# Tariq-Abuhashim/semantic-slam

Measured on AMD Instinct MI355X. Metric: Mvoxels/sec integrated, 512³ grid @ 640×480 depth; achieved HBM GB/s %peak, higher is better.
Workload: dtype f32

## Files before the change

### semantic_slam_amd/csrc/tsdf_capi.hip

```cpp
#include "../../include/tsdf_hip.h"

#include <hip/hip_runtime.h>

#include <algorithm>
#include <cmath>
#include <cstdarg>
#include <cstdio>
#include <cstdlib>
#include <cstring>
#include <new>
#include <string>
#include <unordered_map>
#include <vector>

#include "pose_math.h"
#include "host_derive.h"
#include "host_copy.h"
#include "frame_store.h"
#include "tsdf_kernels.hip.h"
#include "tsdf_multiframe.hip.h"
#include "tsdf_labels.hip.h"
#include "tsdf_colour.hip.h"
#include "tsdf_extract.hip.h"
#ifdef TSDF_EXPERIMENTS
#include "tsdf_experiments.hip.h"
#endif

namespace {

thread_local std::string g_last_error;

int fail(int code, const char *fmt, ...)
{
    char buf[512];
    va_list ap;
    va_start(ap, fmt);
    vsnprintf(buf, sizeof buf, fmt, ap);
    va_end(ap);
    g_last_error = buf;
    return code;
}

#define HIP_TRY(expr)                                                                          \
    do {                                                                                       \
        hipError_t _e = (expr);                                                                \
        if (_e != hipSuccess)                                                                  \
            return fail(TSDF_ERR_HIP, "%s failed: %s (%s:%d)", #expr, hipGetErrorString(_e),   \
                        __FILE__, __LINE__);                                                   \
    } while (0)

constexpr int kStageSlots = 3;

#ifdef TSDF_EXPERIMENTS
constexpr bool kExperiments = true;
#else
constexpr bool kExperiments = false;
#endif

#ifndef TSDF_BRICK_NT
#define TSDF_BRICK_NT 0
#endif
constexpr bool kBrickNT = TSDF_BRICK_NT != 0;
constexpr size_t kClaimBlockBytes = (tsdfk::kCounterBytes + sizeof(tsdfk::ClassPoseTable) + 255) / 256 * 256;
#ifndef TSDF_WEDGE_MODE
#define TSDF_WEDGE_MODE 0
#endif
constexpr int kWedgeMode = TSDF_WEDGE_MODE;

}

struct tsdf_volume {
    tsdf_config cfg;
    float base2world_inv[16];
    float last_cam2base[16];
    int64_t n_vox;
    float *d_tsdf;
    float *d_weight;
    hipStream_t own_stream;
    hipStream_t stream;
    tsdf_store::FrameStore *store;
    hipStream_t copy_stream;
    hipEvent_t flush_done[2];
    int flush_parity;
    int table_slot;
    int defer_n;
    hipEvent_t pend_copied;
    int pend_count;
    int pend_slot[tsdfk::kMaxFramesPerLaunch], pend_mask_slot[tsdfk::kMaxFramesPerLaunch];
    const float *pend_depth[tsdfk::kMaxFramesPerLaunch];
    struct tsdf_batch *owner;
    struct tsdf_group *group_owner;
    bool in_flush;
    float pend_c2b[16 * tsdfk::kMaxFramesPerLaunch];
    const uint8_t *pend_mask[tsdfk::kMaxFramesPerLaunch];
    int variant;
    tsdfk::FramePose *h_frames[kStageSlots];
    tsdfk::FramePose *d_frames[kStageSlots];
    hipEvent_t frames_done[kStageSlots];
    bool frames_used[kStageSlots];
    int frames_next;
    uint16_t *d_label;
    float *d_fp, *d_bp;
    float prob_thd;
    uint32_t *d_colour;
    uint8_t *d_rgb[kStageSlots];
    uint8_t *h_rgb[kStageSlots];
    hipEvent_t rgb_done[kStageSlots];
    bool rgb_used[kStageSlots];
    int rgb_next;
    uint32_t *d_flags;
    size_t n_flags;
    int nseg;
    int chunks_per_slice;
    bool flat;
    int brick_q, brick_r, brick_s;
    int tile;
    bool fine_tables = false;
    bool flags_known_zero;
    unsigned int *d_super;
    size_t super_words;
    uint4 *d_work;
    size_t work_entries;
    int64_t work_nsuper, work_bucket_supers;
    int work_wedge_mode = -1;
    unsigned int *d_shortcut_stats;
    unsigned long long *d_claims, *h_claims;
    hipEvent_t claims_done;
    hipStream_t pre_stream = nullptr, rb_stream = nullptr;
    int rb_parity = -1;
    hipEvent_t pre_done[2] = {nullptr, nullptr}, list_free[2] = {nullptr, nullptr}, seq_ready = nullptr;
    int list_parity = 0;
    bool list_used[2] = {false, false};
    bool pipeline_ok = false;
    bool claims_pending, claims_known;
    double claims_total;
    double claim_fraction;
    int launches_unclassified;
    void *d_scratch;
    size_t scratch_bytes;
    uint8_t *d_wg_class;
    size_t wg_class_bytes;
    void *d_list;
    size_t list_bytes;
};

constexpr int kBatchSideStreams = 4;

struct tsdf_batch {
    int device;
    std::vector<tsdf_volume *> vols;
    hipStream_t stream;
    tsdfk::IntegrateParams *h_params[kStageSlots];
    tsdfk::IntegrateParams *d_params[kStageSlots];
    tsdfk::FramePose *h_poses[kStageSlots];
    tsdfk::FramePose *d_poses[kStageSlots];
    hipEvent_t slot_done[kStageSlots];
    bool slot_used[kStageSlots];
    int slot_next;
    int2 *d_slice_map;
    int total_slices, max_blocks;
    int2 *d_group_map;
    int total_groups;
    std::vector<int> group_s;
    float2 *d_tiles;
    size_t tiles_per_object;
    uint8_t *d_wg_class;
    uint8_t *d_brick_class;
    size_t brick_class_bytes;
    float *d_depth_pool;
    uint8_t *d_mask_pool;
    std::vector<float> pend_c2b;
    std::vector<const uint8_t *> pend_mask;
    int pend_count;
    bool in_flush;
    hipStream_t side[kBatchSideStreams];
    hipEvent_t side_done[kBatchSideStreams];
    hipEvent_t collected;
};

namespace {

int flush_pending(tsdf_volume *v);
int fail(int code, const char *fmt, ...);
int batch_flush(tsdf_batch *b);
int group_flush(tsdf_group *g);
int batch_collect(tsdf_batch *b, const float *depth_dev, const uint8_t *const *masks_dev, const float cam2world[16]);

int bind_device(tsdf_volume *v, bool flush = true)
{
    HIP_TRY(hipSetDevice(v->cfg.device));
    if (v->owner && !v->in_flush) {
        int rc = batch_flush(v->owner);
        if (rc) return rc;
    }
    if (v->group_owner && !v->in_flush) {
        int rc = group_flush(v->group_owner);
        if (rc) return rc;
    }
    if (flush && v->pend_count > 0 && !v->in_flush) return flush_pending(v);
    return TSDF_OK;
}

int store_slot(tsdf_volume *v, tsdf_store::SlotClass *c, hipStream_t first_user, int *index, void **dev)
{
    hipError_t e = tsdf_store::slot_acquire(v->store, c, v, first_user, false, index, dev);
    if (e == hipSuccess && *index < 0) {
        if (v->pend_count > 0 && !v->in_flush) {
            int rc = flush_pending(v);
            if (rc) return rc;
        }
        e = tsdf_store::slot_acquire(v->store, c, v, first_user, true, index, dev);
    }
    if (e != hipSuccess) return fail(TSDF_ERR_HIP, "frame store: %s", hipGetErrorString(e));
    return TSDF_OK;
}

int store_release(tsdf_volume *v, tsdf_store::SlotClass *c, const int *idx, int n)
{
    hipEvent_t *evt = &v->flush_done[v->flush_parity];
    HIP_TRY(hipEventRecord(*evt, v->stream));
    tsdf_store::slots_release_after(v->store, c, idx, n, evt, v);
    return TSDF_OK;
}

void store_next_pass(tsdf_volume *v) { v->flush_parity ^= 1; }

int tables_begin(tsdf_volume *v, float2 **tiles, hipStream_t first_user = nullptr)
{
    void *dev = nullptr;
    hipError_t e = tsdf_store::slot_acquire(v->store, &v->store->tables, v, first_user ? first_user : v->stream, true, &v->table_slot, &dev);
    if (e != hipSuccess) return fail(TSDF_ERR_HIP, "frame store (tile tables): %s", hipGetErrorString(e));
    *tiles = static_cast<float2 *>(dev);
    return TSDF_OK;
}

int tables_end(tsdf_volume *v)
{
    if (v->table_slot < 0) return TSDF_OK;
    const int slot = v->table_slot;
    v->table_slot = -1;
    return store_release(v, &v->store->tables, &slot, 1);
}

using tsdf_host::brick_shape_ok;

void choose_brick_for(const tsdf_config &c, int &bq, int &br, int &bs)
{
#ifdef TSDF_EXPERIMENTS
// ... 77 lines not shown

size_t tile_table_elems_host(int tiles_w, int tiles_h)
{
    return (size_t)tile_levels_host(tiles_w) * tile_levels_host(tiles_h) * tiles_w * tiles_h;
}

bool tiles_fit(const tsdfk::IntegrateParams &p) { return (int64_t)p.tiles_w * p.tiles_h <= 16384; }

constexpr int64_t kFineTileMinVoxels = 10000000;
thread_local bool g_create_for_batch = false;
int tile_edge_for(const tsdf_config &c)
{
    const int64_t n = (int64_t)c.dim_x * c.dim_y * (int64_t)(c.z_end - c.z_begin);
    const int64_t fine_tiles = (int64_t)((c.im_width + 7) / 8) * ((c.im_height + 7) / 8);
    return (!g_create_for_batch && n >= kFineTileMinVoxels && fine_tiles <= tsdfk::kTileLdsEntries) ? 8 : 16;
}

constexpr int64_t kFineLevelMinVoxels = 64000000;
bool fine_tables_for(const tsdf_config &c, int tile)
{
    const int64_t n = (int64_t)c.dim_x * c.dim_y * (int64_t)(c.z_end - c.z_begin);
    bool on = tile == 8 && n >= kFineLevelMinVoxels;
#ifdef TSDF_EXPERIMENTS
    if (const char *e = std::getenv("TSDF_FINE_TILES")) on = tile == 8 && std::atoi(e) != 0;
#endif
    return on;
}

constexpr int64_t kClassifyMinVoxels = 48000000;
bool classify_one_frame(const tsdf_volume *v, int64_t launch_voxels)
{
    if (v->variant == 7) return false;
    return v->variant == 8 || (kExperiments && v->variant >= 11 && v->variant <= 13) || launch_voxels >= kClassifyMinVoxels;
}

int build_tile_tables(hipStream_t stream, const tsdf_config &c, const tsdfk::IntegrateParams &p, const float *const *depth,
                      const uint8_t *const *masks, int n, float2 *tables, unsigned long long *zero_me = nullptr, float2 *fine = nullptr,
                      bool beside_a_launch = false)
{
    const size_t per = tile_table_elems_host(p.tiles_w, p.tiles_h);
    if (fine != nullptr && (p.tile_inv != 0.125f || n > tsdfk::kMaxFramesPerLaunch))
        return fail(TSDF_ERR_INVALID, "build_tile_tables: fine tables go with 8-pixel tiles, one launch at a time");
    for (int k = 0; k < n; k += tsdfk::kMaxFramesPerLaunch) {
        const int m = std::min(tsdfk::kMaxFramesPerLaunch, n - k);
        tsdfk::TileSummaryParams tp;
        for (int f = 0; f < tsdfk::kMaxFramesPerLaunch; ++f) {
            tp.depth[f] = depth[k + (f < m ? f : 0)];
            tp.mask[f] = masks ? masks[k + (f < m ? f : 0)] : nullptr;
        }
        tp.tiles = tables + (size_t)k * per;
        tp.H = c.im_height; tp.W = c.im_width; tp.tiles_w = p.tiles_w; tp.tiles_h = p.tiles_h;
        tp.max_depth = c.max_depth;
        tp.fine = fine; tp.fw = p.fine_w; tp.fh = p.fine_h;
        if (p.tile_inv == 0.0625f) {
            const int strips = ((p.tiles_w + 3) / 4) * p.tiles_h;
            hipLaunchKernelGGL(tsdfk::depth_tile_summary<16>, dim3((unsigned)((strips + 3) / 4), m), dim3(64, 4), 0, stream, tp);
        } else {
            const int strips = ((p.tiles_w + 7) / 8) * p.tiles_h;
            hipLaunchKernelGGL(tsdfk::depth_tile_summary<8>, dim3((unsigned)((strips + 3) / 4), m), dim3(64, 4), 0, stream, tp);
        }
        if (p.tiles_w * p.tiles_h <= tsdfk::kTileLdsEntries) {
            const unsigned threads = (p.tiles_w * p.tiles_h > 2048 && !beside_a_launch) ? 1024 : 256;
            const unsigned fine_blocks = fine ? ((unsigned)(p.fine_w * p.fine_h) + threads - 1) / threads : 0u;
            hipLaunchKernelGGL(tsdfk::tile_sparse_table, dim3((unsigned)tile_levels_host(p.tiles_w) + fine_blocks, m), dim3(threads), 0, stream, tp.tiles,
                               p.tiles_w, p.tiles_h, k == 0 ? zero_me : (unsigned long long *)nullptr, fine, p.fine_w, p.fine_h);
        } else {
            if (zero_me && k == 0) HIP_TRY(hipMemsetAsync(zero_me, 0, tsdfk::kCounterBytes, stream));
            hipLaunchKernelGGL(tsdfk::tile_sparse_table_scan, dim3((unsigned)tile_levels_host(p.tiles_w), m), dim3(256), 0, stream, tp.tiles,
                               p.tiles_w, p.tiles_h);
            if (fine)
                hipLaunchKernelGGL(tsdfk::fine_tile_levels, dim3((unsigned)((p.fine_w * p.fine_h + 255) / 256), m), dim3(256), 0, stream, fine, p.fine_w, p.fine_h);
        }
    }
    HIP_TRY(hipGetLastError());
    return TSDF_OK;
}

int launch_masked_bricks(tsdf_volume *v, tsdfk::IntegrateParams &p)
{
    const int blocks = (p.brick_groups * p.bricks_per_group + 3) / 4, nz = (p.nz + p.brick_s - 1) / p.brick_s;
    float2 *tiles = nullptr;
    int rc0 = tables_begin(v, &tiles);
    if (rc0) return rc0;
    const size_t n_bricks = (size_t)blocks * nz * 4;
    if (v->wg_class_bytes < n_bricks) {
        if (v->d_wg_class) HIP_TRY(hipFree(v->d_wg_class));
        v->d_wg_class = nullptr;
        v->wg_class_bytes = 0;
        HIP_TRY(hipMalloc((void **)&v->d_wg_class, n_bricks));
        v->wg_class_bytes = n_bricks;
    }
    const float *d = p.depth;
    const uint8_t *m = p.mask;
    int rc = build_tile_tables(v->stream, v->cfg, p, &d, &m, 1, tiles);
    if (rc) return rc;
    tsdfk::FramePose pose;
    pose_from_params(pose, p);
    pose.tiles = tiles;
    hipLaunchKernelGGL(tsdfk::classify_bricks, dim3((unsigned)((n_bricks + 255) / 256)), dim3(256), 0, v->stream, p, pose,
                       v->d_wg_class, blocks, nz);
    p.wg_class = v->d_wg_class;
    hipLaunchKernelGGL((tsdfk::integrate_single_bricks<kBrickNT>), dim3(blocks, 1, nz), dim3(64, 4, 1), 0, v->stream, p, pose);
    HIP_TRY(hipGetLastError());
    return tables_end(v);
}


bool shipped_variant(int variant) { return variant == 0 || variant == 1 || variant == 3 || variant == 7 || variant == 8; }

int drop_summary(tsdf_volume *v)
{
    if (v->flags_known_zero || v->n_flags == 0) return TSDF_OK;
    HIP_TRY(hipMemsetAsync(v->d_flags, 0, v->n_flags * sizeof(uint32_t), v->stream));
    v->flags_known_zero = true;
    return TSDF_OK;
}

int rebuild_summary(tsdf_volume *v)
{
    if (v->n_flags == 0 || v->n_vox == 0) return TSDF_OK;
    const int nz = v->cfg.z_end - v->cfg.z_begin;
    const int qps = (int)((int64_t)v->cfg.dim_x * v->cfg.dim_y / 4);
    dim3 block(64, 4, 1), grid((v->chunks_per_slice + 3) / 4, 1, nz);
    hipLaunchKernelGGL(tsdfk::recompute_flags, grid, block, 0, v->stream, v->d_tsdf, v->d_weight, v->d_flags, qps,
                       v->chunks_per_slice);
    HIP_TRY(hipGetLastError());
    v->flags_known_zero = false;
    return TSDF_OK;
}

int launch_multi(tsdf_volume *v, const float *const *depth_dev, const uint8_t *const *masks_dev, const float *c2b, int n,
                 const uint16_t *const *label_ims = nullptr, const float *const *score_ims = nullptr, hipEvent_t inputs_ready = nullptr);

double claims_read_back(const tsdf_volume *v)
{
    double claimed = 0.0;
    for (int b = 0; b < tsdfk::kListBuckets; ++b) {
        const unsigned long long w = v->h_claims[(size_t)b * (tsdfk::kBucketStride / sizeof(unsigned long long)) + 1];
        claimed += (double)(w >> 32) + (double)(w & 0xffffffffull);
    }
    return v->claims_total > 0 ? claimed / v->claims_total : 0.0;
}

#ifdef TSDF_EXPERIMENTS
bool experiment_variant(int variant);
void experiment_adjust(const tsdf_volume *v, bool labels, bool *classify, int *z_fastest);
int launch_integrate_experiment(tsdf_volume *v, const float *depth_dev, const uint8_t *mask_dev, const float *c2b);
int launch_multi_experiment(tsdf_volume *v, tsdfk::MultiParamsInline &mi, const float *const *depth_dev, const uint8_t *const *masks_dev,
                            const float *c2b, int n, bool labels, bool any_mask, bool classify, bool *handled, double *claims_total);
int launch_single_experiment(tsdf_volume *v, tsdfk::IntegrateParams &common, tsdfk::FramePose &pose, const float *depth_dev,
                             const float *c2b, bool *handled);
#endif

int launch_integrate(tsdf_volume *v, const float *depth_dev, const uint8_t *mask_dev,
                     const float *c2b)
{
    const tsdf_config &c = v->cfg;
    const int nz = c.z_end - c.z_begin;
    if (nz == 0) return TSDF_OK;
    std::memcpy(v->last_cam2base, c2b, sizeof v->last_cam2base);
#ifdef TSDF_EXPERIMENTS
    if (c.dim_x % 4 == 0 && (v->variant == 2 || (v->variant >= 16 && !mask_dev))) return launch_integrate_experiment(v, depth_dev, mask_dev, c2b);
#endif
    if (c.dim_x % 4 != 0 || v->variant == 1) {
        int rc = drop_summary(v);
        if (rc) return rc;
        const tsdfk::IntegrateParams p = make_params(v, depth_dev, mask_dev, c2b, 1);
        dim3 block(64, 4, 1), grid((c.dim_x + 63) / 64, (c.dim_y + 3) / 4, nz);
        if (mask_dev) hipLaunchKernelGGL((tsdfk::integrate_scalar<true>), grid, block, 0, v->stream, p);
        else hipLaunchKernelGGL((tsdfk::integrate_scalar<false>), grid, block, 0, v->stream, p);
        HIP_TRY(hipGetLastError());
        return TSDF_OK;
    }
    if (v->flat) {
        return launch_multi(v, &depth_dev, mask_dev ? &mask_dev : nullptr, c2b, 1);
    }
    tsdfk::IntegrateParams p = make_params(v, depth_dev, mask_dev, c2b, 4);
    v->flags_known_zero = false;
    const dim3 block(64, 4, 1), grid((p.xgroups + 63) / 64, (p.dim_y + 7) / 8, p.nz);
    if (mask_dev) {
        if (classify_one_frame(v, v->n_vox) && tiles_fit(p) && p.brick_q > 0 && (!kExperiments || v->variant != 11)) {
            int rc = launch_masked_bricks(v, p);
            if (rc) return rc;
        } else {
#ifdef TSDF_EXPERIMENTS
            if (v->variant == 11 && classify_one_frame(v, v->n_vox) && tiles_fit(p)) return launch_integrate_experiment(v, depth_dev, mask_dev, c2b);
#endif
            hipLaunchKernelGGL((tsdfk::integrate_tile<2, true>), grid, block, 0, v->stream, p);
        }
    } else {
        hipLaunchKernelGGL((tsdfk::integrate_tile<2, false>), grid, block, 0, v->stream, p);
    }
    HIP_TRY(hipGetLastError());
    return TSDF_OK;
}

void compose_cam2base(const tsdf_volume *v, const float *cam2world, float *c2b)
{
    tsdf_host::multiply_matrix(v->base2world_inv, cam2world, c2b);
}

int launch_multi(tsdf_volume *v, const float *const *depth_dev, const uint8_t *const *masks_dev,
                 const float *c2b, int n, const uint16_t *const *label_ims, const float *const *score_ims, hipEvent_t inputs_ready)
{
    const tsdf_config &c = v->cfg;
    const int nz = c.z_end - c.z_begin;
    if (nz == 0 || n == 0) return TSDF_OK;
    auto fill_pose = [&](tsdfk::FramePose &fp, int f) {
        pose_from_params(fp, make_params(v, depth_dev[f], masks_dev ? masks_dev[f] : nullptr, c2b + 16 * f, 4));
        fp.label_im = label_ims ? label_ims[f] : nullptr;
        fp.score_im = label_ims ? score_ims[f] : nullptr;
    };
    const dim3 block(64, 4, 1);
    if (n == 1 && !label_ims) {
        tsdfk::IntegrateParams common = make_params(v, depth_dev[0], nullptr, c2b, 4);
        tsdfk::FramePose pose;
        fill_pose(pose, 0);
        std::memcpy(v->last_cam2base, c2b, sizeof v->last_cam2base);
        v->flags_known_zero = false;
#ifdef TSDF_EXPERIMENTS
        {
            bool handled = false;
            int rc = launch_single_experiment(v, common, pose, depth_dev[0], c2b, &handled);
            if (rc || handled) return rc;
        }
#endif
        if (v->flat && pose.mask != nullptr && classify_one_frame(v, v->n_vox) && tiles_fit(common) && common.brick_q > 0) {
            tsdfk::IntegrateParams cp = make_params(v, depth_dev[0], pose.mask, c2b, 4);
            return launch_masked_bricks(v, cp);
        }
        if (v->flat) {
            dim3 grid((v->chunks_per_slice + 3) / 4, 1, nz);
            hipLaunchKernelGGL((tsdfk::integrate_multi_single<true, true>), grid, block, 0, v->stream, common, pose);
        } else {
            dim3 grid((common.xgroups + 63) / 64, (c.dim_y + 3) / 4, nz);
            hipLaunchKernelGGL((tsdfk::integrate_multi_single<true, false>), grid, block, 0, v->stream, common, pose);
        }
        HIP_TRY(hipGetLastError());
        return TSDF_OK;
    }
    std::memcpy(v->last_cam2base, c2b + 16 * (n - 1), sizeof v->last_cam2base);
    v->flags_known_zero = false;
    tsdfk::MultiParamsInline mi;
    mi.common = make_params(v, depth_dev[0], nullptr, c2b, 4);
    mi.n_frames = n;
    for (int f = 0; f < n; ++f) fill_pose(mi.frames[f], f);
    for (int f = n; f < tsdfk::kMaxFramesPerLaunch; ++f) mi.frames[f] = mi.frames[0];
    mi.labels.label = v->d_label; mi.labels.fp = v->d_fp; mi.labels.bp = v->d_bp; mi.labels.prob_thd = v->prob_thd;
    bool any_mask = false;
    for (int f = 0; f < n && masks_dev; ++f) any_mask = any_mask || masks_dev[f] != nullptr;

    if (v->claims_pending) {
        const hipError_t qe = hipEventQuery(v->claims_done);
        if (qe == hipSuccess) {
            v->claim_fraction = claims_read_back(v);
            v->claims_pending = false;
            v->claims_known = true;
        } else if (qe == hipErrorNotReady) {
            (void)hipGetLastError();
        } else {
            v->claims_pending = false;
            v->claims_known = false;
            (void)hipGetLastError();
            return fail(TSDF_ERR_HIP, "claims read-back: hipEventQuery failed: %s", hipGetErrorString(qe));
        }
    }
    bool classify = tiles_fit(mi.common) && v->variant != 7 && mi.common.brick_q > 0;
    mi.z_fastest = 2;
#ifdef TSDF_EXPERIMENTS
    experiment_adjust(v, label_ims != nullptr, &classify, &mi.z_fastest);
#endif
    const bool forced = v->variant == 8 || (kExperiments && v->variant >= 11 && v->variant <= 13);
    if (classify && !forced) classify = !v->claims_known || v->claim_fraction >= 0.10 || v->launches_unclassified >= 7;
    v->launches_unclassified = classify ? 0 : v->launches_unclassified + 1;
    const bool count_claims = classify && !v->claims_pending;
    if (classify && !v->d_claims) {
        unsigned long long *dc = nullptr;
        unsigned char *hc = nullptr;
        hipEvent_t ev[6] = {nullptr, nullptr, nullptr, nullptr, nullptr, nullptr};
        hipError_t e = hipMalloc((void **)&dc, 2 * kClaimBlockBytes);
        if (e == hipSuccess) e = hipHostMalloc((void **)&hc, tsdfk::kCounterBytes, hipHostMallocDefault);
        for (int i = 0; i < 6 && e == hipSuccess; ++i) e = hipEventCreateWithFlags(&ev[i], hipEventDisableTiming);
        if (e != hipSuccess) {
            for (int i = 0; i < 6; ++i) if (ev[i]) (void)hipEventDestroy(ev[i]);
            if (hc) (void)hipHostFree(hc);
            if (dc) (void)hipFree(dc);
            return fail(TSDF_ERR_HIP, "claim counters: %s", hipGetErrorString(e));
        }
        v->d_claims = reinterpret_cast<decltype(v->d_claims)>(dc);
        v->h_claims = reinterpret_cast<decltype(v->h_claims)>(hc);
        v->claims_done = ev[0];
        v->pre_done[0] = ev[1]; v->pre_done[1] = ev[2]; v->list_free[0] = ev[3]; v->list_free[1] = ev[4]; v->seq_ready = ev[5];
    }
    const int P = v->pipeline_ok ? v->list_parity : 0;
    unsigned long long *const claims_p = classify ? v->d_claims + (size_t)P * (kClaimBlockBytes / sizeof(unsigned long long)) : nullptr;
    bool pipelined = classify && inputs_ready != nullptr && v->pipeline_ok;
#ifdef TSDF_EXPERIMENTS
    if (!shipped_variant(v->variant) || std::getenv("TSDF_NO_PIPELINE")) pipelined = false;
#endif
    if (pipelined && !v->pre_stream) {
        hipStream_t a = nullptr, b = nullptr;
        int prio = 0;
#ifdef TSDF_EXPERIMENTS
        if (std::getenv("TSDF_PRE_PRIORITY")) { int lo = 0, hi = 0; (void)hipDeviceGetStreamPriorityRange(&lo, &hi); prio = hi; }
#endif
        hipError_t e = hipStreamCreateWithPriority(&a, hipStreamNonBlocking, prio);
        if (e == hipSuccess) e = hipStreamCreateWithFlags(&b, hipStreamNonBlocking);
        if (e != hipSuccess) {
            if (a) (void)hipStreamDestroy(a);
            return fail(TSDF_ERR_HIP, "side streams: %s", hipGetErrorString(e));
        }
        v->pre_stream = a;
        v->rb_stream = b;
    }
    const hipStream_t ps = pipelined ? v->pre_stream : v->stream;
    if (pipelined) {
        HIP_TRY(hipStreamWaitEvent(ps, inputs_ready, 0));
        if (v->list_used[P]) HIP_TRY(hipStreamWaitEvent(ps, v->list_free[P], 0));
        if (v->rb_parity == P) HIP_TRY(hipStreamWaitEvent(ps, v->claims_done, 0));
    } else if (classify && v->rb_parity == P) {
        HIP_TRY(hipStreamWaitEvent(v->stream, v->claims_done, 0));
    }
    if (count_claims) mi.common.claim_counter = claims_p + 1;
    if (classify) {
        const size_t per_frame = tile_table_elems_host(mi.common.tiles_w, mi.common.tiles_h);
        float2 *tiles = nullptr;
        int rc = tables_begin(v, &tiles, ps);
        if (rc) return rc;
        float2 *fine = v->fine_tables ? tiles + (size_t)tsdfk::kMaxFramesPerLaunch * per_frame : nullptr;
        rc = build_tile_tables(ps, c, mi.common, depth_dev, masks_dev, n, tiles, claims_p, fine, pipelined);
        if (rc) return rc;
        mi.common.fine = fine;
        for (int f = 0; f < n; ++f) mi.frames[f].tiles = tiles + (size_t)f * per_frame;
        for (int f = n; f < tsdfk::kMaxFramesPerLaunch; ++f) mi.frames[f] = mi.frames[0];
    }
    const int nz_groups = (nz + mi.common.brick_s - 1) / mi.common.brick_s;
    double claims_total = 0.0;
    bool launched = false, listed = false;
#ifdef TSDF_EXPERIMENTS
    {
        int rc = launch_multi_experiment(v, mi, depth_dev, masks_dev, c2b, n, label_ims != nullptr, any_mask, classify, &launched, &claims_total);
        if (rc) return rc;
    }
// ... 2066 lines not shown
```

### semantic_slam_amd/csrc/tsdf_kernels.hip.h

```cpp
#pragma once
#include <hip/hip_runtime.h>
#include <stdint.h>

namespace tsdfk {

struct IntegrateParams {
    const float *depth;
    const uint8_t *mask;
    float *tsdf;
    float *weight;
    float fx, fy, cx, cy;
    float rx0, rx1, rx2;
    float ry0, ry1, ry2;
    float rz0, rz1, rz2;
    float tx, ty, tz;
    float ox, oy, oz;
    float vs, trunc, max_depth;
    int dim_x, dim_y;
    int nz, z_begin;
    int H, W;
    int xgroups;
    uint32_t *flags;
    int nseg;
    int quads_per_row, quads_per_slice, chunks_per_slice;
    int brick_q, brick_r, brick_s, bricks_per_group, brick_groups;
    int brick_q_magic, brick_per_magic;
    int fast_ok;
    int trunc_fast;
    float cz_margin;
    int tiles_w, tiles_h;
    float tile_inv;
    const float2 *fine = nullptr;
    int fine_w = 0, fine_h = 0;
    float px_margin_u, px_margin_v;
    unsigned int *shortcut_stats;
    float cz_short, cz_pad;
    unsigned long long *claim_counter;
    const uint8_t *wg_class;
};

struct RowTerms {
    float x1, x2, y1, y2, z1, z2;
};

__device__ __forceinline__ RowTerms row_terms(const IntegrateParams &p, int gy, int gz)
{
    float by = p.oy + (float)gy * p.vs;
    float bz = p.oz + (float)gz * p.vs;
    float dy = by - p.ty;
    float dz = bz - p.tz;
    RowTerms r;
    r.x1 = p.rx1 * dy; r.x2 = p.rx2 * dz;
    r.y1 = p.ry1 * dy; r.y2 = p.ry2 * dz;
    r.z1 = p.rz1 * dy; r.z2 = p.rz2 * dz;
    return r;
}

template <bool MASKED>
__device__ __forceinline__ bool voxel_dist(const IntegrateParams &p, const RowTerms &r, int gx,
                                           float &dist)
{
    float bx = p.ox + (float)gx * p.vs;
    float dx = bx - p.tx;
    float pcx = p.rx0 * dx + r.x1 + r.x2;
    float pcy = p.ry0 * dx + r.y1 + r.y2;
    float pcz = p.rz0 * dx + r.z1 + r.z2;
    if (pcz <= 0.0f) return false;

    float pu = roundf(p.fx * (pcx / pcz) + p.cx);
    float pv = roundf(p.fy * (pcy / pcz) + p.cy);
    if (!(pu >= 0.0f && pu < (float)p.W && pv >= 0.0f && pv < (float)p.H)) return false;
    int pix = (int)pv * p.W + (int)pu;

    float d = p.depth[pix];
    if (MASKED) d = d * (p.mask[pix] >= 128 ? 1.0f : 0.0f);
    if (d <= 0.0f || d > p.max_depth) return false;

    float diff = d - pcz;
    if (diff <= -p.trunc) return false;
    dist = fminf(1.0f, diff / p.trunc);
    return true;
}

template <bool MASKED>
__global__ __launch_bounds__(256) void integrate_scalar(IntegrateParams p)
{
    const int gx = blockIdx.x * 64 + threadIdx.x;
    const int gy = blockIdx.y * 4 + threadIdx.y;
    const int lz = blockIdx.z;
    if (gx >= p.dim_x || gy >= p.dim_y) return;
    const int gz = p.z_begin + lz;
    const RowTerms r = row_terms(p, gy, gz);
    float dist;
    const bool upd = voxel_dist<MASKED>(p, r, gx, dist);
    if (__ballot(upd) == 0ull) return;
    if (!upd) return;
    const size_t at = ((size_t)lz * p.dim_y + gy) * (size_t)p.dim_x + (size_t)gx;
    const float w_old = p.weight[at];
    const float w_new = w_old + 1.0f;
    p.weight[at] = w_new;
    p.tsdf[at] = (p.tsdf[at] * w_old + dist) / w_new;
}

typedef float v2f __attribute__((ext_vector_type(2)));

__device__ __forceinline__ float refined_rcp(float d)
{
    const float r0 = __builtin_amdgcn_rcpf(d);
    const float e0 = __builtin_fmaf(-d, r0, 1.0f);
    return __builtin_fmaf(e0, r0, r0);
}

__device__ __forceinline__ float fast_div_r(float n, float d, float r1)
{
    const float q0 = n * r1;
    const float e1 = __builtin_fmaf(-d, q0, n);
    const float q1 = __builtin_fmaf(e1, r1, q0);
    const float e2 = __builtin_fmaf(-d, q1, n);
    return __builtin_fmaf(e2, r1, q1);
}

__device__ __forceinline__ v2f fast_div2(v2f n, float d)
{
    const float r1 = refined_rcp(d);
    const v2f R = {r1, r1}, D = {d, d};
    const v2f q0 = n * R;
    const v2f e1 = __builtin_elementwise_fma(-D, q0, n);
    const v2f q1 = __builtin_elementwise_fma(e1, R, q0);
    const v2f e2 = __builtin_elementwise_fma(-D, q1, n);
    return __builtin_elementwise_fma(e2, R, q1);
}

__device__ __forceinline__ int round_half_up_i32(float u)
{
    int r;
    asm("v_cvt_rpi_i32_f32 %0, %1" : "=v"(r) : "v"(u));
    return r;
}

#define TSDF_FAST_D_MIN 8.6736174e-19f

typedef float v4f __attribute__((ext_vector_type(4)));
typedef unsigned int v4u __attribute__((ext_vector_type(4)));

template <bool NT>
__device__ __forceinline__ float4 vol_load(const float *p)
{
    if constexpr (NT) {
        v4f v = __builtin_nontemporal_load(reinterpret_cast<const v4f *>(p));
        return make_float4(v.x, v.y, v.z, v.w);
    } else {
        return *reinterpret_cast<const float4 *>(p);
    }
}
template <bool NT>
__device__ __forceinline__ void vol_store(float *p, float4 v)
{
    if constexpr (NT) {
        v4f q = {v.x, v.y, v.z, v.w};
        __builtin_nontemporal_store(q, reinterpret_cast<v4f *>(p));
    } else {
        *reinterpret_cast<float4 *>(p) = v;
    }
}

__device__ __forceinline__ float gather_f32(const float *__restrict__ base, uint32_t px)
{
    return *reinterpret_cast<const float *>(reinterpret_cast<const char *>(base) + (px << 2));
}

__device__ __forceinline__ int pixel_index24(int iv, int W, int iu)
{
    return (int)(__umul24((unsigned)iv, (unsigned)W) + (unsigned)iu);
}

template <int R, int MASKED>
__device__ __forceinline__ void integrate_tile_body(const IntegrateParams &p, const int bx, const int by, const int lz)
{
    const int gz = p.z_begin + lz;
    const int xg = bx * 64 + threadIdx.x;
    const int gy0 = (by * 4 + threadIdx.y) * R;
    if (xg >= p.xgroups || gy0 >= p.dim_y) return;
    const size_t row0 = ((size_t)lz * p.dim_y + gy0) * (size_t)p.dim_x + (size_t)xg * 4;
    const size_t flag0 = ((size_t)lz * p.dim_y + gy0) * (size_t)p.nseg + bx;

    uint32_t fl[R];
    float4 t4[R], w4[R];
#pragma unroll
    for (int r = 0; r < R; ++r) {
        fl[r] = gy0 + r < p.dim_y ? p.flags[flag0 + (size_t)r * p.nseg] : 0u;
        t4[r] = make_float4(1.f, 1.f, 1.f, 1.f);
        w4[r] = make_float4(0.f, 0.f, 0.f, 0.f);
    }

    float ax[4], ay[4], az[4];
#pragma unroll
    for (int j = 0; j < 4; ++j) {
        float bx = p.ox + (float)(xg * 4 + j) * p.vs;
        float dx = bx - p.tx;
        ax[j] = p.rx0 * dx; ay[j] = p.ry0 * dx; az[j] = p.rz0 * dx;
    }
    const float bz = p.oz + (float)gz * p.vs;
    const float dz = bz - p.tz;
    const float x2 = p.rx2 * dz, y2 = p.ry2 * dz, z2 = p.rz2 * dz;

    float pcz[R][4], dval[R][4];
    bool geo[R][4];
    int pixel[R][4];
#pragma unroll
    for (int r = 0; r < R; ++r) {
        const float dy = (p.oy + (float)(gy0 + r) * p.vs) - p.ty;
        const float z1 = p.rz1 * dy;
#pragma unroll
        for (int j = 0; j < 4; ++j) pcz[r][j] = az[j] + z1 + z2;
    }
    const float cmin = fminf(fminf(pcz[0][0], pcz[0][3]), fminf(pcz[R - 1][0], pcz[R - 1][3]));
    const float cmax = fmaxf(fmaxf(pcz[0][0], pcz[0][3]), fmaxf(pcz[R - 1][0], pcz[R - 1][3]));
    const bool unsafe = !(cmin > p.cz_margin) & !(cmax < -p.cz_margin);
    const bool fast = p.fast_ok != 0 && __ballot(unsafe) == 0ull;
    if (fast) {
        const v2f F = {p.fx, p.fy}, C = {p.cx, p.cy};
        const bool front = cmin > p.cz_margin;
#pragma unroll
        for (int r = 0; r < R; ++r) {
            const bool row_ok = gy0 + r < p.dim_y;
            const float dy = (p.oy + (float)(gy0 + r) * p.vs) - p.ty;
            const v2f XY1 = {p.rx1 * dy, p.ry1 * dy};
            const v2f XY2 = {x2, y2};
#pragma unroll
            for (int j = 0; j < 4; ++j) {
                const v2f A = {ax[j], ay[j]};
                const v2f n = A + XY1 + XY2;
                const float cz = pcz[r][j];
                const v2f uv = F * fast_div2(n, cz) + C;
                const int iu = round_half_up_i32(uv.x), iv = round_half_up_i32(uv.y);
                const bool ok = row_ok & front & (uv.x > -0.5f) & (uv.y > -0.5f) &
                                ((unsigned)iu < (unsigned)p.W) & ((unsigned)iv < (unsigned)p.H);
                geo[r][j] = ok;
                pixel[r][j] = ok ? pixel_index24(iv, p.W, iu) : 0;
            }
        }
    } else {
#pragma unroll
        for (int r = 0; r < R; ++r) {
            const int gy = gy0 + r;
            const bool row_ok = gy < p.dim_y;
            const float by = p.oy + (float)gy * p.vs;
            const float dy = by - p.ty;
            const float x1 = p.rx1 * dy, y1 = p.ry1 * dy;
#pragma unroll
            for (int j = 0; j < 4; ++j) {
                const float cx = ax[j] + x1 + x2;
                const float cy = ay[j] + y1 + y2;
                const float cz = pcz[r][j];
                const float pu = roundf(p.fx * (cx / cz) + p.cx);
                const float pv = roundf(p.fy * (cy / cz) + p.cy);
                const bool ok = row_ok && !(cz <= 0.0f) && pu >= 0.0f && pu < (float)p.W && pv >= 0.0f &&
                                pv < (float)p.H;
                geo[r][j] = ok;
                pixel[r][j] = ok ? (int)pv * p.W + (int)pu : 0;
            }
        }
    }
#pragma unroll
    for (int r = 0; r < R; ++r) {
#pragma unroll
        for (int j = 0; j < 4; ++j) {
            const uint32_t px = (uint32_t)pixel[r][j];
            float d = gather_f32(p.depth, px);
            if (MASKED == 1) d = d * (p.mask[px] >= 128 ? 1.0f : 0.0f);
            dval[r][j] = d;
        }
    }

    float diff[R][4];
    bool upd[R][4], rowany[R], bandr[R];
    bool any = false, band = false;
#pragma unroll
    for (int r = 0; r < R; ++r) {
        rowany[r] = false;
        bandr[r] = false;
#pragma unroll
        for (int j = 0; j < 4; ++j) {
            const float d = dval[r][j];
            const float df = d - pcz[r][j];
            diff[r][j] = df;
            const bool u = geo[r][j] & !((d <= 0.0f) | (d > p.max_depth)) & !(df <= -p.trunc);
            upd[r][j] = u;
            rowany[r] |= u;
            bandr[r] |= u & !(df >= p.trunc);
        }
        band |= bandr[r];
        any |= rowany[r];
    }
    if (__ballot(any) == 0ull) return;
    if (!any) return;

#pragma unroll
    for (int r = 0; r < R; ++r) {
        if (rowany[r]) {
            w4[r] = vol_load<true>(p.weight + row0 + (size_t)r * p.dim_x);
            if (!(fl[r] & 1u)) t4[r] = vol_load<true>(p.tsdf + row0 + (size_t)r * p.dim_x);
        }
    }
    float dist[R][4];
    if (__ballot(band) != 0ull) {
#pragma unroll
        for (int r = 0; r < R; ++r)
#pragma unroll
            for (int j = 0; j < 4; ++j) dist[r][j] = fminf(1.0f, diff[r][j] / p.trunc);
    } else {
#pragma unroll
        for (int r = 0; r < R; ++r)
#pragma unroll
            for (int j = 0; j < 4; ++j) dist[r][j] = 1.0f;
    }

#pragma unroll
    for (int r = 0; r < R; ++r) {
        if (fl[r] == 3u && __ballot(bandr[r]) == 0ull) {
            if (rowany[r]) {
                const float4 w = w4[r];
                vol_store<true>(p.weight + row0 + (size_t)r * p.dim_x,
                                make_float4(upd[r][0] ? w.x + 1.0f : w.x, upd[r][1] ? w.y + 1.0f : w.y,
                                            upd[r][2] ? w.z + 1.0f : w.z, upd[r][3] ? w.w + 1.0f : w.w));
            }
            continue;
        }
        float tv[4] = {t4[r].x, t4[r].y, t4[r].z, t4[r].w};
        float wv[4] = {w4[r].x, w4[r].y, w4[r].z, w4[r].w};
        float num[4], wn[4];
        bool need = false;
#pragma unroll
        for (int j = 0; j < 4; ++j) {
            wn[j] = wv[j] + 1.0f;
            num[j] = tv[j] * wv[j] + dist[r][j];
            need |= upd[r][j] && !(num[j] == wn[j] && wn[j] < 3.0e38f && wn[j] > 0.0f);
        }
        float nt[4];
        if (__ballot(rowany[r] && need) != 0ull) {
#pragma unroll
            for (int j = 0; j < 4; ++j) nt[j] = num[j] / wn[j];
        } else {
#pragma unroll
            for (int j = 0; j < 4; ++j) nt[j] = 1.0f;
        }
        bool changed = false, notone = false;
#pragma unroll
        for (int j = 0; j < 4; ++j) {
            const float newt = upd[r][j] ? nt[j] : tv[j];
            changed |= __float_as_uint(newt) != __float_as_uint(tv[j]);
            notone |= upd[r][j] && __float_as_uint(newt) != 0x3f800000u;
            tv[j] = newt;
            wv[j] = upd[r][j] ? wn[j] : wv[j];
        }
        if ((fl[r] & 1u) && __ballot(notone) != 0ull) {
            if (notone) p.flags[flag0 + (size_t)r * p.nseg] = fl[r] & 2u;
        }
        const bool store_t = __ballot(rowany[r] && changed) != 0ull;
        if (rowany[r]) {
            if (store_t) vol_store<true>(p.tsdf + row0 + (size_t)r * p.dim_x, make_float4(tv[0], tv[1], tv[2], tv[3]));
            vol_store<true>(p.weight + row0 + (size_t)r * p.dim_x, make_float4(wv[0], wv[1], wv[2], wv[3]));
        }
    }
}

template <int R, bool MASKED>
__global__ __launch_bounds__(256) void integrate_tile(IntegrateParams p)
{
    integrate_tile_body<R, MASKED ? 1 : 0>(p, blockIdx.x, blockIdx.y, blockIdx.z);
}

__device__ __forceinline__ uint32_t hash32(uint64_t x)
{
    x ^= x >> 33; x *= 0xff51afd7ed558ccdull; x ^= x >> 33; x *= 0xc4ceb9fe1a85ec53ull; x ^= x >> 33;
    return (uint32_t)x;
}

__global__ __launch_bounds__(256) void selftest_fastdiv(uint64_t seed, uint64_t n_samples, float fx, float cx,
                                                        unsigned long long *mismatch, float *first_bad)
{
    const uint64_t stride = (uint64_t)gridDim.x * blockDim.x;
    for (uint64_t i = (uint64_t)blockIdx.x * blockDim.x + threadIdx.x; i < n_samples; i += stride) {
        const uint32_t h0 = hash32(seed + 3 * i), h1 = hash32(seed + 3 * i + 1), h2 = hash32(seed + 3 * i + 2);
        const uint32_t mode = h2 & 7u;
        uint32_t dm = h0 & 0x7fffffu;
        if (mode == 1) dm = 0x7fffffu; else if (mode == 2) dm = 0u; else if (mode == 3) dm &= 0x7u;
        const uint32_t de = 127u - 60u + (h0 >> 23) % 121u;
        const float d = __uint_as_float((de << 23) | dm);
        uint32_t ne = (mode >= 6) ? ((h1 >> 23) % 190u) : (de - 12u + (h1 >> 23) % 24u);
        if (ne > 127u + 60u) ne = 127u + 60u;
        uint32_t nm = h1 & 0x7fffffu;
        if (mode == 4) nm = 0x7fffffu; else if (mode == 5) nm = dm;
        float n0 = __uint_as_float(((h2 >> 3) & 1u) << 31 | (ne << 23) | nm);
        float n1 = __uint_as_float(((h2 >> 4) & 1u) << 31 | (((ne + (h2 >> 8) % 5u) % 188u) << 23) | (h2 >> 9));
        if ((h2 >> 5 & 31u) == 0u) n0 = 0.0f;
        const v2f nn = {n0, n1};
        const v2f q = fast_div2(nn, d);
        const float r0 = n0 / d, r1 = n1 / d;
        bool bad0 = __float_as_uint(q.x) != __float_as_uint(r0);
        bool bad1 = __float_as_uint(q.y) != __float_as_uint(r1);
        auto same_pixel = [&](float qa, float qb) {
            const float ua = fx * qa + cx, ub = fx * qb + cx;
            return round_half_up_i32(ua) == round_half_up_i32(ub) && (ua > -0.5f) == (ub > -0.5f);
        };
        if (bad0 && fabsf(r0) < 2.2737368e-13f) bad0 = !same_pixel(q.x, r0);
        if (bad1 && fabsf(r1) < 2.2737368e-13f) bad1 = !same_pixel(q.y, r1);
        if (bad0 || bad1) {
            if (atomicAdd(mismatch, 1ull) == 0ull) {
                first_bad[0] = bad0 ? n0 : n1; first_bad[1] = d; first_bad[2] = bad0 ? q.x : q.y;
                first_bad[3] = bad0 ? r0 : r1;
            }
        }
    }
}

__global__ __launch_bounds__(256) void selftest_fastdiv_band(uint64_t seed, uint64_t n_samples, unsigned long long *mismatch,
                                                             float *first_bad)
{
    const uint64_t stride = (uint64_t)gridDim.x * blockDim.x;
    for (uint64_t i = (uint64_t)blockIdx.x * blockDim.x + threadIdx.x; i < n_samples; i += stride) {
        const uint32_t h0 = hash32(seed + 3 * i), h1 = hash32(seed + 3 * i + 1), h2 = hash32(seed + 3 * i + 2);
        const uint32_t mode = h2 & 7u;
        uint32_t dm = h0 & 0x7fffffu;
        if (mode == 1) dm = 0x7fffffu; else if (mode == 2) dm = 0u; else if (mode == 3) dm &= 0x7u;
        const uint32_t de = 127u - 20u + (h0 >> 23) % 41u;
        const float d = __uint_as_float((de << 23) | dm);
        uint32_t ne = 127u - 81u + (h1 >> 23) % 142u;
        if (mode >= 6) ne = de - 2u + (h1 >> 23) % 5u;
        if (ne > 127u + 60u) ne = 127u + 60u;
        uint32_t nm = h1 & 0x7fffffu;
        if (mode == 4) nm = 0x7fffffu; else if (mode == 5) nm = dm;
        if (ne == 127u + 60u) nm = 0u;
        float n = __uint_as_float((((h2 >> 3) & 1u) << 31) | (ne << 23) | nm);
        if (((h2 >> 5) & 63u) == 0u) n = 0.0f;
        if (((h2 >> 5) & 63u) == 1u) n = __uint_as_float(0x7fc00000u | (h2 >> 12));
        const float q = fast_div_r(n, d, refined_rcp(d));
        const float r = n / d;
        const bool same = __float_as_uint(q) == __float_as_uint(r) || (q != q && r != r);
        if (!same) {
            if (atomicAdd(mismatch, 1ull) == 0ull) { first_bad[0] = n; first_bad[1] = d; first_bad[2] = q; first_bad[3] = r; }
        }
    }
}

__global__ __launch_bounds__(256) void selftest_round(unsigned long long *mismatch, float *first_bad)
{
    const uint64_t stride = (uint64_t)gridDim.x * blockDim.x;
    const uint64_t n_pos = 0x4B800001ull, n_neg = 0x3F000000ull;
    for (uint64_t i = (uint64_t)blockIdx.x * blockDim.x + threadIdx.x; i < n_pos + n_neg; i += stride) {
        const uint32_t bits = i < n_pos ? (uint32_t)i : (0x80000000u + (uint32_t)(i - n_pos));
        const float u = __uint_as_float(bits);
        if (!(u > -0.5f)) continue;
        const int want = (int)roundf(u);
        const int got = round_half_up_i32(u);
        if (got != want) {
            if (atomicAdd(mismatch, 1ull) == 0ull) { first_bad[0] = u; first_bad[1] = (float)got; first_bad[2] = (float)want; first_bad[3] = 0.f; }
        }
    }
}

template <bool NT>
__global__ __launch_bounds__(256) void stream_rmw(float *tsdf, float *weight, size_t n_quads, float one,
                                                  float zero)
{
    const size_t stride = (size_t)gridDim.x * blockDim.x;
    for (size_t q = (size_t)blockIdx.x * blockDim.x + threadIdx.x; q < n_quads; q += stride) {
        float4 t = vol_load<NT>(tsdf + 4 * q);
        float4 w = vol_load<NT>(weight + 4 * q);
        t.x *= one; t.y *= one; t.z *= one; t.w *= one;
        w.x += zero; w.y += zero; w.z += zero; w.w += zero;
        vol_store<NT>(tsdf + 4 * q, t);
        vol_store<NT>(weight + 4 * q, w);
    }
}

__global__ __launch_bounds__(256) void recompute_flags(const float *tsdf, const float *weight, uint32_t *flags,
                                                       int quads_per_slice, int chunks_per_slice)
{
    const int chunk = blockIdx.x * 4 + threadIdx.y;
    if (chunk >= chunks_per_slice) return;
    const int q = chunk * 64 + threadIdx.x;
    const size_t base = ((size_t)blockIdx.z * quads_per_slice + q) * 4;
    bool ones = true, sane = true;
    if (q < quads_per_slice) {
        const float4 t = *reinterpret_cast<const float4 *>(tsdf + base);
        const float4 w = *reinterpret_cast<const float4 *>(weight + base);
        ones = __float_as_uint(t.x) == 0x3f800000u && __float_as_uint(t.y) == 0x3f800000u &&
               __float_as_uint(t.z) == 0x3f800000u && __float_as_uint(t.w) == 0x3f800000u;
        sane = w.x >= 0.0f && w.x < 3.0e38f && w.y >= 0.0f && w.y < 3.0e38f && w.z >= 0.0f && w.z < 3.0e38f &&
               w.w >= 0.0f && w.w < 3.0e38f;
    }
    const uint32_t f = (__ballot(!ones) == 0ull ? 1u : 0u) | (__ballot(!sane) == 0ull ? 2u : 0u);
    if (threadIdx.x == 0) flags[(size_t)blockIdx.z * chunks_per_slice + chunk] = f;
}

__global__ __launch_bounds__(256) void depth_u16_to_f32(const uint16_t *raw, float *out, int H, int W,
                                                        float scale, int row_step, int col_step)
{
    const int n = H * W;
    for (int i = blockIdx.x * blockDim.x + threadIdx.x; i < n; i += gridDim.x * blockDim.x) {
        const int r = i / W, c = i - r * W;
        const bool keep = (r % row_step == 0) && (c % col_step == 0);
        out[i] = (keep ? (float)raw[i] : 0.0f) * scale;
    }
}

__device__ __forceinline__ void atomic_min_float(float *addr, float v)
{
    if (__float_as_int(v) >= 0) atomicMin(reinterpret_cast<int *>(addr), __float_as_int(v));
    else atomicMax(reinterpret_cast<unsigned int *>(addr), __float_as_uint(v));
}

__global__ __launch_bounds__(256) void object_origin(const float *depth, const uint8_t *mask, int H, int W, float fx,
                                                     float fy, float cx, float cy, float *out)
{
    float mx = 1000.0f, my = 1000.0f, mz = 1000.0f;
    const float ifx = 1.0f / fx, ify = 1.0f / fy;
    const int n = H * W;
    for (int i = blockIdx.x * blockDim.x + threadIdx.x; i < n; i += gridDim.x * blockDim.x) {
        float z = depth[i];
        if (mask != nullptr) z = z * (mask[i] >= 128 ? 1.0f : 0.0f);
        if (z <= 0.0f) continue;
// ... 26 lines not shown
```

Before: 390,400.

## Alternate z-sweep direction and keep tail slices cache-resident across frames

Each integrate launch now alternates its z traversal direction. The last window of slices touched (sized to a 512 MB budget) uses plain loads and stores instead of nontemporal ones, so those slices stay in the last-level cache (MALL). The next frame sweeps in the opposite direction and starts on those cached slices, which is meant to cut HBM traffic for a working set that exceeds the cache. This adds per-thread branching on the cache mode, and the gain depends on the actual cache capacity.

Measured after the change: 411,400 (median of 6 runs). +5.4%, better.

```diff
diff --git a/semantic_slam_amd/csrc/tsdf_capi.hip b/semantic_slam_amd/csrc/tsdf_capi.hip
--- a/semantic_slam_amd/csrc/tsdf_capi.hip
+++ b/semantic_slam_amd/csrc/tsdf_capi.hip
@@ -94,6 +94,7 @@
     float pend_c2b[16 * tsdfk::kMaxFramesPerLaunch];
     const uint8_t *pend_mask[tsdfk::kMaxFramesPerLaunch];
     int variant;
+    int sweep_parity;
     tsdfk::FramePose *h_frames[kStageSlots];
     tsdfk::FramePose *d_frames[kStageSlots];
     hipEvent_t frames_done[kStageSlots];
@@ -477,6 +478,25 @@
                              const float *c2b, bool *handled);
 #endif
 
+constexpr int64_t kWindowBytes = 512ll << 20;
+
+void set_sweep(tsdf_volume *v, tsdfk::IntegrateParams &p)
+{
+    int64_t window = kWindowBytes;
+    bool forward_only = false;
+#ifdef TSDF_EXPERIMENTS
+    if (const char *e = std::getenv("TSDF_MALL_WINDOW_MB")) window = (int64_t)std::atoi(e) << 20;
+    forward_only = std::getenv("TSDF_SWEEP_FORWARD") && std::atoi(std::getenv("TSDF_SWEEP_FORWARD")) != 0;
+    p.head_plain_loads = std::getenv("TSDF_HEAD_PLAIN_LOADS") && std::atoi(std::getenv("TSDF_HEAD_PLAIN_LOADS")) != 0;
+#endif
+    const int64_t slice_bytes = 8 * (int64_t)p.dim_x * p.dim_y;
+    const int w = (int)std::min<int64_t>(p.nz, window / slice_bytes);
+    p.sweep_reverse = forward_only ? 0 : v->sweep_parity;
+    v->sweep_parity ^= 1;
+    p.cache_lo = p.sweep_reverse ? 0 : p.nz - w;
+    p.cache_hi = p.sweep_reverse ? w : p.nz;
+}
+
 int launch_integrate(tsdf_volume *v, const float *depth_dev, const uint8_t *mask_dev,
                      const float *c2b)
 {
@@ -511,9 +531,11 @@
 #ifdef TSDF_EXPERIMENTS
             if (v->variant == 11 && classify_one_frame(v, v->n_vox) && tiles_fit(p)) return launch_integrate_experiment(v, depth_dev, mask_dev, c2b);
 #endif
+            set_sweep(v, p);
             hipLaunchKernelGGL((tsdfk::integrate_tile<2, true>), grid, block, 0, v->stream, p);
         }
     } else {
+        set_sweep(v, p);
         hipLaunchKernelGGL((tsdfk::integrate_tile<2, false>), grid, block, 0, v->stream, p);
     }
     HIP_TRY(hipGetLastError());
diff --git a/semantic_slam_amd/csrc/tsdf_kernels.hip.h b/semantic_slam_amd/csrc/tsdf_kernels.hip.h
--- a/semantic_slam_amd/csrc/tsdf_kernels.hip.h
+++ b/semantic_slam_amd/csrc/tsdf_kernels.hip.h
@@ -1,6 +1,7 @@
 #pragma once
 #include <hip/hip_runtime.h>
 #include <stdint.h>
+#include <type_traits>
 
 namespace tsdfk {
 
@@ -37,6 +38,11 @@
     float cz_short, cz_pad;
     unsigned long long *claim_counter;
     const uint8_t *wg_class;
+    int sweep_reverse = 0;
+    int cache_lo = 0, cache_hi = 0;
+#ifdef TSDF_EXPERIMENTS
+    int head_plain_loads = 0;
+#endif
 };
 
 struct RowTerms {
@@ -164,6 +170,17 @@
     }
 }
 
+template <bool NT>
+__device__ __forceinline__ float4 vol_load_p(std::integral_constant<bool, NT>, const float *p) { return vol_load<NT>(p); }
+__device__ __forceinline__ float4 vol_load_p(bool nt, const float *p) { return nt ? vol_load<true>(p) : vol_load<false>(p); }
+template <bool NT>
+__device__ __forceinline__ void vol_store_p(std::integral_constant<bool, NT>, float *p, float4 v) { vol_store<NT>(p, v); }
+__device__ __forceinline__ void vol_store_p(bool nt, float *p, float4 v)
+{
+    if (nt) vol_store<true>(p, v);
+    else vol_store<false>(p, v);
+}
+
 __device__ __forceinline__ float gather_f32(const float *__restrict__ base, uint32_t px)
 {
     return *reinterpret_cast<const float *>(reinterpret_cast<const char *>(base) + (px << 2));
@@ -175,7 +192,8 @@
 }
 
 template <int R, int MASKED>
-__device__ __forceinline__ void integrate_tile_body(const IntegrateParams &p, const int bx, const int by, const int lz)
+__device__ __forceinline__ void integrate_tile_body(const IntegrateParams &p, const int bx, const int by, const int lz,
+                                                    const bool lnt, const bool snt)
 {
     const int gz = p.z_begin + lz;
     const int xg = bx * 64 + threadIdx.x;
@@ -299,8 +317,9 @@
 #pragma unroll
     for (int r = 0; r < R; ++r) {
         if (rowany[r]) {
-            w4[r] = vol_load<true>(p.weight + row0 + (size_t)r * p.dim_x);
-            if (!(fl[r] & 1u)) t4[r] = vol_load<true>(p.tsdf + row0 + (size_t)r * p.dim_x);
+            const float *wp = p.weight + row0 + (size_t)r * p.dim_x, *tp = p.tsdf + row0 + (size_t)r * p.dim_x;
+            w4[r] = vol_load_p(lnt, wp);
+            if (!(fl[r] & 1u)) t4[r] = vol_load_p(lnt, tp);
         }
     }
     float dist[R][4];
@@ -316,59 +335,74 @@
             for (int j = 0; j < 4; ++j) dist[r][j] = 1.0f;
     }
 
-#pragma unroll
-    for (int r = 0; r < R; ++r) {
-        if (fl[r] == 3u && __ballot(bandr[r]) == 0ull) {
+    auto store_rows = [&](auto snt_c) {
+    #pragma unroll
+        for (int r = 0; r < R; ++r) {
+            if (fl[r] == 3u && __ballot(bandr[r]) == 0ull) {
+                if (rowany[r]) {
+                    const float4 w = w4[r];
+                    vol_store_p(snt_c, p.weight + row0 + (size_t)r * p.dim_x,
+                                    make_float4(upd[r][0] ? w.x + 1.0f : w.x, upd[r][1] ? w.y + 1.0f : w.y,
+                                                upd[r][2] ? w.z + 1.0f : w.z, upd[r][3] ? w.w + 1.0f : w.w));
+                }
+                continue;
+            }
+            float tv[4] = {t4[r].x, t4[r].y, t4[r].z, t4[r].w};
+            float wv[4] = {w4[r].x, w4[r].y, w4[r].z, w4[r].w};
+            float num[4], wn[4];
+            bool need = false;
+    #pragma unroll
+            for (int j = 0; j < 4; ++j) {
+                wn[j] = wv[j] + 1.0f;
+                num[j] = tv[j] * wv[j] + dist[r][j];
+                need |= upd[r][j] && !(num[j] == wn[j] && wn[j] < 3.0e38f && wn[j] > 0.0f);
+            }
+            float nt[4];
+            if (__ballot(rowany[r] && need) != 0ull) {
+    #pragma unroll
+                for (int j = 0; j < 4; ++j) nt[j] = num[j] / wn[j];
+            } else {
+    #pragma unroll
+                for (int j = 0; j < 4; ++j) nt[j] = 1.0f;
+            }
+            bool changed = false, notone = false;
+    #pragma unroll
+            for (int j = 0; j < 4; ++j) {
+                const float newt = upd[r][j] ? nt[j] : tv[j];
+                changed |= __float_as_uint(newt) != __float_as_uint(tv[j]);
+                notone |= upd[r][j] && __float_as_uint(newt) != 0x3f800000u;
+                tv[j] = newt;
+                wv[j] = upd[r][j] ? wn[j] : wv[j];
+            }
+            if ((fl[r] & 1u) && __ballot(notone) != 0ull) {
+                if (notone) p.flags[flag0 + (size_t)r * p.nseg] = fl[r] & 2u;
+            }
+            const bool store_t = __ballot(rowany[r] && changed) != 0ull;
             if (rowany[r]) {
-                const float4 w = w4[r];
-                vol_store<true>(p.weight + row0 + (size_t)r * p.dim_x,
-                                make_float4(upd[r][0] ? w.x + 1.0f : w.x, upd[r][1] ? w.y + 1.0f : w.y,
-                                            upd[r][2] ? w.z + 1.0f : w.z, upd[r][3] ? w.w + 1.0f : w.w));
-            }
-            continue;
-        }
-        float tv[4] = {t4[r].x, t4[r].y, t4[r].z, t4[r].w};
-        float wv[4] = {w4[r].x, w4[r].y, w4[r].z, w4[r].w};
-        float num[4], wn[4];
-        bool need = false;
-#pragma unroll
-        for (int j = 0; j < 4; ++j) {
-            wn[j] = wv[j] + 1.0f;
-            num[j] = tv[j] * wv[j] + dist[r][j];
-            need |= upd[r][j] && !(num[j] == wn[j] && wn[j] < 3.0e38f && wn[j] > 0.0f);
-        }
-        float nt[4];
-        if (__ballot(rowany[r] && need) != 0ull) {
-#pragma unroll
-            for (int j = 0; j < 4; ++j) nt[j] = num[j] / wn[j];
-        } else {
-#pragma unroll
-            for (int j = 0; j < 4; ++j) nt[j] = 1.0f;
-        }
-        bool changed = false, notone = false;
-#pragma unroll
-        for (int j = 0; j < 4; ++j) {
-            const float newt = upd[r][j] ? nt[j] : tv[j];
-            changed |= __float_as_uint(newt) != __float_as_uint(tv[j]);
-            notone |= upd[r][j] && __float_as_uint(newt) != 0x3f800000u;
-            tv[j] = newt;
-            wv[j] = upd[r][j] ? wn[j] : wv[j];
-        }
-        if ((fl[r] & 1u) && __ballot(notone) != 0ull) {
-            if (notone) p.flags[flag0 + (size_t)r * p.nseg] = fl[r] & 2u;
-        }
-        const bool store_t = __ballot(rowany[r] && changed) != 0ull;
-        if (rowany[r]) {
-            if (store_t) vol_store<true>(p.tsdf + row0 + (size_t)r * p.dim_x, make_float4(tv[0], tv[1], tv[2], tv[3]));
-            vol_store<true>(p.weight + row0 + (size_t)r * p.dim_x, make_float4(wv[0], wv[1], wv[2], wv[3]));
-        }
+                if (store_t) vol_store_p(snt_c, p.tsdf + row0 + (size_t)r * p.dim_x, make_float4(tv[0], tv[1], tv[2], tv[3]));
+                vol_store_p(snt_c, p.weight + row0 + (size_t)r * p.dim_x, make_float4(wv[0], wv[1], wv[2], wv[3]));
+            }
+        }
+    };
+    if constexpr (MASKED == 1) {
+        if (snt) store_rows(std::true_type{});
+        else store_rows(std::false_type{});
+    } else {
+        store_rows(snt);
     }
 }
 
 template <int R, bool MASKED>
 __global__ __launch_bounds__(256) void integrate_tile(IntegrateParams p)
 {
-    integrate_tile_body<R, MASKED ? 1 : 0>(p, blockIdx.x, blockIdx.y, blockIdx.z);
+    const int lz = p.sweep_reverse ? p.nz - 1 - (int)blockIdx.z : (int)blockIdx.z;
+    const bool cached = lz >= p.cache_lo && lz < p.cache_hi;
+#ifdef TSDF_EXPERIMENTS
+    const bool lnt = !cached && !p.head_plain_loads;
+#else
+    const bool lnt = !cached;
+#endif
+    integrate_tile_body<R, MASKED ? 1 : 0>(p, blockIdx.x, blockIdx.y, lz, lnt, !cached);
 }
 
 __device__ __forceinline__ uint32_t hash32(uint64_t x)
```
